# UBCMOCCA/mocca_envs

Hardware: AMD Instinct MI355X
Metric: env-steps/sec, Walker3DCustomEnv-v0 @ 4096 envs, 1/2/4/8 MI355X (higher is better)
Workload: dtype f32; 1 GPU; Walker3DCustomEnv-v0, 4096 envs/GPU, flat ground, U(-1,1) action tape, auto-reset; max_rows=48, max_contacts=12, envs_per_gpu=4096, parallelism=independent env shards x1, no collective, preroll_steps=6008

## Files before the change

mocca_envs_amd/csrc/mocca_device.h:

```cpp
#pragma once

#include <hip/hip_runtime.h>
#include <stdint.h>

#include "mocca_model.h"
#include "mocca_philox.h"
#include "topo_walker3d.h"
#include "topo_cassie.h"
#include "topo_walker2d.h"
#include "topo_crab2d.h"
#include "topo_laikago.h"

#define DI __device__ __forceinline__

#ifndef MOCCA_NS
#define MOCCA_NS mocca
#endif
#ifndef MOCCA_MAXR
#define MOCCA_MAXR 48
#endif
#ifndef MOCCA_COMPACT
#define MOCCA_COMPACT 0
#endif

// ... 11 lines not shown
#define STAMP(k) do {} while (0)
#define STAMP_BEGIN do {} while (0)
#endif

#define MOCCA_AS_CONST __attribute__((address_space(4)))
typedef const MOCCA_AS_CONST MoccaModel* ModelP;
typedef float f4_t __attribute__((ext_vector_type(4)));
typedef const MOCCA_AS_CONST f4_t* CF4P;

#ifndef MOCCA_PRIO_T3
#define MOCCA_PRIO_T3 12
#define MOCCA_PRIO_T2 7
#define MOCCA_PRIO_T1 4
#endif
constexpr int MAXR = MOCCA_MAXR;
constexpr int MAXC = MAXR >= 64 ? 20 : (MAXR >= 36 ? 12 : MAXR / 3);
constexpr bool COMPACT = MOCCA_COMPACT != 0;
constexpr bool ALT_SWEEPS = MAXR >= 64;
constexpr int DYN_STRIDE = 96;
constexpr int TERRAIN_STRIDE = 128;

#ifndef MOCCA_LDS_PAD
#define MOCCA_LDS_PAD 0
#endif
enum : int {
  L_Q = 0,
  L_QD = 24,
  L_TAU = 48,
  L_NU = 72,
  L_BASE = 100,
  L_WARM = 116,
  L_FEET = 156,
  L_PLANK = 168,
  L_JVEL = 168,
  L_Q0 = 184,
  L_V = 216,
  SVS = 20, SV_V = 6, SV_C = 12, SV_UU = 18, SV_INVD = 19,
  L_B0 = L_V + 0,
  L_SV = L_V + 48,
#if MOCCA_COMPACT
  L_ROWD = L_B0,
  L_CT = L_V + 488,
  L_P = L_CT + 16 * MAXC,
  L_M = L_P + 132,
  L_RT = L_M,
  L_GP = L_M + 264,
  GP_FLOATS = 192,
  L_OBS = L_GP,
  L_CAND = L_GP + GP_FLOATS,
  L_ABA_END = L_M + 792,
  L_A = L_V,
  L_J = L_V + 488,
  L_XL = L_V,
  L_SOLVER_END = (L_J + 28 * (MAXR + 1) > L_A + MAXR * MAXR ? L_J + 28 * (MAXR + 1) : L_A + MAXR * MAXR),
  L_TOTAL = (L_ABA_END > L_SOLVER_END ? L_ABA_END : L_SOLVER_END) + MOCCA_LDS_PAD,
#else
  L_A0 = L_V + 488,
  L_GP = L_V + 520,
  L_OBS = L_V + 520,
  L_CT = L_V + 656,
  GP_FLOATS = L_CT - L_GP,
  L_ROWD = L_CT + 16 * MAXC,
  L_RT = L_ROWD + 48,
  L_M = L_RT + 264,
  L_P = L_M + 792,
  L_ABA_END = L_P + 132,
  L_CAND = L_ABA_END,
  L_A = L_V,
  L_J = (L_V + 960 > L_RT ? L_V + 960 : L_RT),
  L_XL = L_V,
  L_TOTAL = L_V + MAXR * MAXR + 28 + MOCCA_LDS_PAD,
#endif
};
static_assert(L_ABA_END <= L_TOTAL, "ABA view must fit");
static_assert(L_SV % 4 == 0 && SVS % 4 == 0 && SVS >= 16, "joint records live in the body records, 16-byte aligned");
static_assert(L_J + (MAXR + 1) * 28 <= L_TOTAL, "Jacobian rows (+ dummy) must fit the tail of the A region");
static_assert(L_J % 4 == 0 && L_V % 4 == 0 && L_RT % 4 == 0 && L_CT % 4 == 0, "16-byte alignment of broadcast rows");
static_assert(MAXR % 2 == 0 && 3 * MAXC <= MAXR, "friction rows sit on the top 2 MAXC lanes of the row range, odd lane = second tangent");
static_assert(L_PLANK + 12 * MOCCA_MAX_PLANKS <= L_V && L_Q0 + 16 <= L_V, "persistent region overflows into the two-view region");
#if MOCCA_COMPACT
static_assert(L_TOTAL * 4 <= 8192 || MOCCA_LDS_PAD > 0, "more than 8 KB of LDS per wave: fewer than 20 waves per CU (5 per SIMD)");
static_assert(L_J >= L_SV + 22 * SVS, "J rows are written while S, V, 1/D are still being read");
static_assert(L_CAND + (MOCCA_MAX_PAIRS + 1) / 2 <= L_ABA_END && L_RT + 264 <= L_GP, "frames, geom points and the candidate list live under the link inertias");
#else
static_assert(L_TOTAL * 4 <= 10240 || MOCCA_LDS_PAD > 0 || MAXR > 48, "more than 10 KB of LDS per wave: fewer than 16 waves per CU, the 4096-env batch no longer fits one round");
static_assert(MAXR != 48 || (L_ROWD == L_V + 848 && L_RT == L_V + 896 && L_M == L_V + 1160 && L_P == L_V + 1952 && L_ABA_END == L_V + 2084 && L_J == L_V + 960), "the product's layout is unchanged");
static_assert(COMPACT || L_CAND + (MOCCA_MAX_PAIRS + 1) / 2 <= L_TOTAL, "candidate list behind the ABA view");
static_assert(L_J >= L_RT, "J rows may be written while S, U, 1/D, the factor of IA0 and the contacts are still being read");
#endif

enum : int { C_BA = 0, C_BB = 1, C_SLOT = 2, C_P = 3, C_N = 6, C_DEPTH = 9, C_MU = 10, C_ERP = 11, C_CFM = 12, C_MA = 13, C_MB = 14 };

struct StepArgs {
  const MoccaModel* model;
  float* dyn;
  uint32_t* task;
  float* terrain;
  const float* act;
  float* obs;
  float* rew;
  uint8_t* done;
  int32_t* info;
  const uint8_t* mask;
  int n_envs;
  int obs_dim;
  int auto_reset;
  int eval_mode;
  int random_pose;
  int curriculum;
  int host_retarget;
  int env_offset;
  uint32_t seed_lo, seed_hi;
  const float* curriculum_v;
  const float* eval_mode_v;
  int random_reward;
  const float* gain_v;
  float gain;
  const int32_t* inj_touch;
  const int32_t* inj_target;
  const int32_t* inj_body;
  const float* tape;
  int tape_n;
  int32_t* dbg;
  const float* traj;
  int traj_n;
  double traj_tmax, traj_cstep;
  int prio;
  const float* hf;
  int hf_rows, hf_cols;
  float hf_scale;
  float* final_obs;
  int persist_warm;
  const int32_t* order;
  int pace;
  unsigned long long* pace_acc;
  float* ep_ret;
  float* ep_masks;
  float* ep_bad;
  void* ep_rec;
  float* ep_totals;
  uint32_t ep_serial;
// ... 314 lines not shown
      L[L_SV + SVS * b + SV_UU] = L[L_TAU + b] - jdamp * L[L_QD + b];
    }
  }
}

template <class T, bool FULL>
DI void walk_kinematics(ModelP M, float* L, int lane, unsigned long long ppk) {
  asm volatile("" : "+v"(lane));
  const int b = lane < T::NB ? lane : 0;
  WalkConsts wk;
  walk_consts<FULL>(M, b, wk);
  walk_phase1<T>(L, lane, ppk);
  wsync();
  walk_phase2<T, FULL>(M, L, lane, b, ppk, wk);
}

DI void chol6_factor(const float* A, float* F) {
  float Lm[6][6];
#pragma unroll
  for (int j = 0; j < 6; ++j) {
    float s = A[sym(j, j)];
#pragma unroll
    for (int k = 0; k < j; ++k) s -= Lm[j][k] * Lm[j][k];
    const float id = rsq(s);
    F[sym(j, j)] = id;
#pragma unroll
    for (int i = j + 1; i < 6; ++i) {
      float t = A[sym(i, j)];
#pragma unroll
      for (int k = 0; k < j; ++k) t -= Lm[i][k] * Lm[j][k];
      Lm[i][j] = t * id;
      F[sym(i, j)] = Lm[i][j];
    }
  }
}
DI void chol6_solve(const float* F, const float* b, float* x) {
  float y[6];
#pragma unroll
  for (int j = 0; j < 6; ++j) {
    float t = b[j];
#pragma unroll
    for (int k = 0; k < j; ++k) t -= F[sym(j, k)] * y[k];
    y[j] = t * F[sym(j, j)];
  }
#pragma unroll
  for (int i = 5; i >= 0; --i) {
    float t = y[i];
#pragma unroll
    for (int k = i + 1; k < 6; ++k) t -= F[sym(k, i)] * x[k];
    x[i] = t * F[sym(i, i)];
  }
}

template <class T>
DI void aba_passes(ModelP M, float* L, int lane, unsigned long long ppk, float* Afac) {
  STAMP_BEGIN;
  static_assert(T::MAXW * 8 <= 64, "level does not fit a wave");
  static_assert(T::MAXW == 4 && T::MAXCH <= 4, "level pass is written for <= 4 bodies per level, <= 4 children");
  const int s = lane >> 3, i = lane & 7;
  const int ii = i < 6 ? i : 0;
  float crow[6] = {0, 0, 0, 0, 0, 0}, cpA = 0.0f;
  int bb = 0, o6i = 0, o36 = 0, osv = 0, osvi = 0;
#pragma unroll
  for (int d = T::MAXD; d >= 1; --d) {
#define MOCCA_CONT(sl) (T::clevel(d, sl) < 0 || (d < T::MAXD && T::clevel(d + 1 <= T::MAXD ? d + 1 : d, sl) == T::clevel(d, sl) + 1))
    const bool sv = s == 0 ? T::clevel(d, 0) >= 0 : s == 1 ? T::clevel(d, 1) >= 0 : s == 2 ? T::clevel(d, 2) >= 0 : s == 3 ? T::clevel(d, 3) >= 0 : false;
    const bool valid = sv && i < 6;
    if (d < T::MAXD && MOCCA_CONT(0) && MOCCA_CONT(1) && MOCCA_CONT(2) && MOCCA_CONT(3)) {
      bb -= 1; o6i -= 6; o36 -= 36; osv -= SVS; osvi -= SVS;
    } else {
      const int b = s == 0 ? T::clevel(d, 0) : s == 1 ? T::clevel(d, 1) : s == 2 ? T::clevel(d, 2) : s == 3 ? T::clevel(d, 3) : -1;
      bb = b >= 0 ? b : d;
      o6i = 6 * bb + ii; o36 = 36 * bb + 6 * ii; osv = SVS * bb; osvi = osv + ii;
    }
#undef MOCCA_CONT
    float row[6], S[6], c[6], pAi;
#pragma unroll
    for (int j = 0; j < 6; ++j) { S[j] = L[L_SV + osv + j]; c[j] = L[L_SV + osv + SV_C + j]; }
#define MOCCA_NOMASS(sl) (T::clevel(d, sl) < 0 || T::massless(T::clevel(d, sl)))
    if (MOCCA_NOMASS(0) && MOCCA_NOMASS(1) && MOCCA_NOMASS(2) && MOCCA_NOMASS(3)) {
#pragma unroll
      for (int j = 0; j < 6; ++j) row[j] = crow[j];
      pAi = cpA;
    } else {
#pragma unroll
      for (int j = 0; j < 6; ++j) row[j] = L[L_M + o36 + j] + crow[j];
      pAi = L[L_P + o6i] + cpA;
    }
#undef MOCCA_NOMASS
#pragma unroll
    for (int k = 0; k < T::MAXCH; ++k) {
#define MOCCA_LDS_CHILD(sl) (T::cchild(T::clevel(d, sl), k) != T::ccarry(T::clevel(d, sl)) ? T::cchild(T::clevel(d, sl), k) : -1)
      const int ch = s == 0 ? MOCCA_LDS_CHILD(0) : s == 1 ? MOCCA_LDS_CHILD(1) : s == 2 ? MOCCA_LDS_CHILD(2) : s == 3 ? MOCCA_LDS_CHILD(3) : -1;
      if (MOCCA_LDS_CHILD(0) >= 0 || MOCCA_LDS_CHILD(1) >= 0 || MOCCA_LDS_CHILD(2) >= 0 || MOCCA_LDS_CHILD(3) >= 0) {
        if (ch >= 0) {
#pragma unroll
          for (int j = 0; j < 6; ++j) row[j] += L[L_M + 36 * ch + 6 * ii + j];
          pAi += L[L_P + 6 * ch + ii];
        }
      }
#undef MOCCA_LDS_CHILD
    }
    const float Si = i < 6 ? L[L_SV + osvi] : 0.0f;
    const float Ui = dot6(row, S);
    float dsum = Si * Ui, psum = Si * pAi;
    group8_sum2(dsum, psum);
    float arm = L[L_SV + osv + SV_INVD], unet = L[L_SV + osv + SV_UU];
// ... 15 lines not shown
        "v_fmac_f32_dpp %4, %7, %8 quad_perm:[0,0,0,0] row_mask:0xf bank_mask:0xf\n\t"
        "v_fmac_f32_dpp %5, %7, %8 quad_perm:[1,1,1,1] row_mask:0xf bank_mask:0xf"
        : "+v"(row[0]), "+v"(row[1]), "+v"(row[2]), "+v"(row[3]), "+v"(row[4]), "+v"(row[5]) : "v"(LO), "v"(HI), "v"(nuid));
#pragma unroll
    for (int j = 0; j < 6; ++j) Iac += row[j] * c[j];
    const float pOut = pAi + Iac + uid * u;
#define MOCCA_VIA_LDS(sl) (T::clevel(d, sl) >= 0 && T::ccarry(T::parent(T::clevel(d, sl) >= 0 ? T::clevel(d, sl) : 0)) != T::clevel(d, sl))
    const bool store_m = MOCCA_VIA_LDS(0) || MOCCA_VIA_LDS(1) || MOCCA_VIA_LDS(2) || MOCCA_VIA_LDS(3);
    if (valid) {
      if (store_m) {
#pragma unroll
        for (int j = 0; j < 6; ++j) L[L_M + o36 + j] = row[j];
        L[L_P + o6i] = pOut;
      }
      L[L_SV + osvi + SV_V] = uid;
      if (i == 0) { L[L_SV + osv + SV_INVD] = id; L[L_SV + osv + SV_UU] = u * id; }
    }
#define MOCCA_NEEDZ(sl) (d > 1 && T::clevel(d - 1, sl) >= 0 && !(T::clevel(d, sl) >= 0 && !MOCCA_VIA_LDS(sl)))
    if (MOCCA_NEEDZ(0) || MOCCA_NEEDZ(1) || MOCCA_NEEDZ(2) || MOCCA_NEEDZ(3)) {
      const bool z = s == 0 ? MOCCA_NEEDZ(0) : s == 1 ? MOCCA_NEEDZ(1) : s == 2 ? MOCCA_NEEDZ(2) : MOCCA_NEEDZ(3);
#pragma unroll
      for (int j = 0; j < 6; ++j) crow[j] = z ? 0.0f : row[j];
      cpA = z ? 0.0f : pOut;
    } else {
#pragma unroll
      for (int j = 0; j < 6; ++j) crow[j] = row[j];
      cpA = pOut;
    }
#undef MOCCA_NEEDZ
#undef MOCCA_VIA_LDS
    if (store_m) wsync();
  }
  STAMP(10);
  float abase[6];
  {
    float rowb[6], pb_ = L[L_P + ii];
#pragma unroll
    for (int j = 0; j < 6; ++j) rowb[j] = L[L_M + 6 * ii + j];
#pragma unroll
    for (int k = 0; k < T::MAXCH; ++k) {
      const int ch = T::cchild(0, k);
      if (ch >= 0) {
#pragma unroll
        for (int j = 0; j < 6; ++j) rowb[j] += L[L_M + 36 * ch + 6 * ii + j];
        pb_ += L[L_P + 6 * ch + ii];
      }
    }
    if (lane < 6) {
      float4* dst = reinterpret_cast<float4*>(L + L_B0 + 8 * lane);
      dst[0] = make_float4(rowb[0], rowb[1], rowb[2], rowb[3]);
      dst[1] = make_float4(rowb[4], rowb[5], pb_, 0.0f);
    }
    wsync();
    float IA[21], pA[6];
#pragma unroll
    for (int i = 0; i < 6; ++i) {
      const float4 lo = *reinterpret_cast<const float4*>(L + L_B0 + 8 * i), hi = *reinterpret_cast<const float4*>(L + L_B0 + 8 * i + 4);
      const float rr_[6] = {lo.x, lo.y, lo.z, lo.w, hi.x, hi.y};
#pragma unroll
      for (int j = i; j < 6; ++j) IA[sym(i, j)] = rr_[j];
      pA[i] = hi.z;
    }
    float Ai[21], a0[6];
    chol6_factor(IA, Ai);
    chol6_solve(Ai, pA, a0);
#pragma unroll
    for (int i = 0; i < 21; ++i) Afac[i] = unif(Ai[i]);
#pragma unroll
    for (int i = 0; i < 6; ++i) abase[i] = -a0[i];
  }
  STAMP(11);
  {
    const int b = lane < T::NB ? lane : 0;
    float a[6], qdd = 0;
#pragma unroll
    for (int i = 0; i < 6; ++i) a[i] = abase[i];
#pragma unroll
    for (int k = 0; k < T::MAXD; ++k) {
      const int j = (int)((ppk >> (5 * k)) & 31ull);
      if (j != 0) {
        float U[6], S[6];
#pragma unroll
        for (int i = 0; i < 6; ++i) { a[i] += L[L_SV + SVS * j + SV_C + i]; U[i] = L[L_SV + SVS * j + SV_V + i]; S[i] = L[L_SV + SVS * j + i]; }
        qdd = L[L_SV + SVS * j + SV_UU] - dot6(U, a);
#pragma unroll
        for (int i = 0; i < 6; ++i) a[i] += S[i] * qdd;
      }
    }
    const float dt = M->dt;
    if (lane >= 1 && lane < T::NB) L[L_NU + 5 + b] = L[L_QD + b] + dt * qdd;
    if (lane == 0) {
      float om[3] = {L[L_BASE + 10], L[L_BASE + 11], L[L_BASE + 12]}, vl[3] = {L[L_BASE + 7], L[L_BASE + 8], L[L_BASE + 9]}, wxv[3];
      cross3(om, vl, wxv);
#pragma unroll
      for (int i = 0; i < 3; ++i) {
        L[L_NU + i] = om[i] + dt * a[i];
        L[L_NU + 3 + i] = vl[i] + dt * (a[3 + i] + wxv[i]);
      }
    }
    wsync();
  }
  STAMP(12);
}

DI void plane_space(const float* n, float* t1, float* t2) {
  if (fabsf(n[2]) > 0.70710678f) {
    const float a = n[1] * n[1] + n[2] * n[2], k = rsq(a);
    t1[0] = 0; t1[1] = -n[2] * k; t1[2] = n[1] * k;
    t2[0] = a * k; t2[1] = -n[0] * t1[2]; t2[2] = n[0] * t1[1];
  } else {
    const float a = n[0] * n[0] + n[1] * n[1], k = rsq(a);
    t1[0] = -n[1] * k; t1[1] = n[0] * k; t1[2] = 0;
    t2[0] = -n[2] * t1[1]; t2[1] = n[2] * t1[0]; t2[2] = a * k;
  }
}
DI void fast_sincos(float q, float* s, float* c);
DI void euler_to_mat(float roll, float pitch, float yaw, float* R) {
  float cr, sr, cp, sp, cy, sy;
  fast_sincos(roll, &sr, &cr); fast_sincos(pitch, &sp, &cp); fast_sincos(yaw, &sy, &cy);
  R[0] = cy * cp; R[1] = cy * sp * sr - sy * cr; R[2] = cy * sp * cr + sy * sr;
// ... 150 lines not shown
#pragma unroll 1
        for (int t = 0; t < 2; ++t) {
          const float* a = t == 0 ? v00 : v10;
          const float* b = t == 0 ? v10 : v11;
          float e1[3], e2[3], tn[3];
#pragma unroll
          for (int k = 0; k < 3; ++k) { e1[k] = b[k] - a[k]; e2[k] = v01[k] - a[k]; }
          cross3(e1, e2, tn);
          hf_triangle(C, rad, a, b, v01, tn, rsq(dot3(tn, tn)), gap, n);
        }
      }
  }
  return gap;
}
DI float hf_height_at(const float* hf, int rows, int cols, float sc, float x, float y) {
  const float ox = (float)rows / sc * 0.5f, oy = (float)cols / sc * 0.5f;
  int ix = (int)((x + ox) * sc), iy = (int)((y + oy) * sc);
  ix = ix < 0 ? 0 : (ix > cols - 1 ? cols - 1 : ix);
  iy = iy < 0 ? 0 : (iy > rows - 1 ? rows - 1 : iy);
  return hf[iy * cols + ix];
}

DI float clamp01(float x) { return x < 0.0f ? 0.0f : (x > 1.0f ? 1.0f : x); }
DI void seg_seg(const float* p1, const float* q1, const float* p2, const float* q2, float* c1, float* c2) {
  float d1[3], d2[3], r[3];
#pragma unroll
  for (int k = 0; k < 3; ++k) { d1[k] = q1[k] - p1[k]; d2[k] = q2[k] - p2[k]; r[k] = p1[k] - p2[k]; }
  const float a = dot3(d1, d1), e = dot3(d2, d2), f = dot3(d2, r), EPS = 1e-12f;
  float s, t;
  if (a <= EPS && e <= EPS) { s = t = 0; }
  else if (a <= EPS) { s = 0; t = clamp01(f * rcp(e)); }
  else {
    const float c = dot3(d1, r), ia = rcp(a);
    if (e <= EPS) { t = 0; s = clamp01(-c * ia); }
    else {
      const float b = dot3(d1, d2), den = a * e - b * b;
      s = den > EPS ? clamp01((b * f - c * e) * rcp(den)) : 0.0f;
      t = (b * s + f) * rcp(e);
      if (t < 0) { t = 0; s = clamp01(-c * ia); }
      else if (t > 1) { t = 1; s = clamp01((b - c) * ia); }
    }
  }
#pragma unroll
  for (int k = 0; k < 3; ++k) { c1[k] = p1[k] + d1[k] * s; c2[k] = p2[k] + d2[k] * t; }
}

template <class T>
DI void geom_points(ModelP M, float* L, int lane) {
  static_assert(6 * T::NG <= GP_FLOATS || (T::NPAIR == 0 && !COMPACT), "geom points would overlap the contact records read by the self-collision pass");
  if (lane < 2 * T::NG) {
    const f4_t t = *(CF4P)(M->gp_tab[lane]);
    const int b = __float_as_int(t.w);
    const float pl[3] = {t.x, t.y, t.z};
#pragma unroll
    for (int i = 0; i < 3; ++i) {
      const float4 fr = *reinterpret_cast<const float4*>(L + L_RT + 12 * b + 4 * i);
      L[L_GP + 3 * lane + i] = fr.x * pl[0] + fr.y * pl[1] + fr.z * pl[2] + fr.w;
    }
  }
}

DI void stage_planks(ModelP M, float* L, int lane, const float* ter) {
  if (lane < M->n_planks) {
    const int row = (int)ter[120 + lane];
    const float* ti = ter + 6 * row;
    float Rb[9];
    euler_to_mat(ti[4], ti[5], ti[3], Rb);
    const float cz = M->plank_com_z, dz = -M->plank_half[2] - cz;
#pragma unroll
    for (int i = 0; i < 9; ++i) L[L_PLANK + 12 * lane + i] = Rb[i];
    L[L_PLANK + 12 * lane + 9] = ti[0] + Rb[2] * dz;
    L[L_PLANK + 12 * lane + 10] = ti[1] + Rb[5] * dz;
    L[L_PLANK + 12 * lane + 11] = ti[2] + Rb[8] * dz + cz;
  }
  wsync();
}

struct HeightFieldArgs { const float* data; int rows, cols; float scale; };
struct ContactFlags { int touch0, touch1, target0, target1, touch2, touch3, body_touch, target2, target3; };
DI int cover_targets(int cover, int nsi, int n_planks, int f) { return (cover >> (4 * f + nsi % n_planks)) & 1; }

template <class T, int TASK>
DI ContactFlags collide(ModelP M, float* L, int lane, const float* ter, int next_step_index,
                        int* nc_out, int32_t* dbg, int* nc_wanted, const HeightFieldArgs hfa, int* cover_out = nullptr) {
  STAMP_BEGIN;
  const float mreach = unif(M->contact_margin);
  ContactFlags fl = {0, 0, 0, 0, 0, 0, 0, 0, 0};
  const int maxc = uni(M->max_contacts);
  bool active = false;
  float n[3] = {0, 0, 1}, P[3] = {0, 0, 0}, gap = 1e30f, mu = 0, erp = M->erp, cfm = 0;
  int body = -1, slot = lane, cover_k = -1 , gfoot = -1, gtorso = 0;
  unsigned bmask = 0u;
  if (lane < T::NSLOT) {
    const f4_t st = *(CF4P)(M->slot_tab[lane]);
    const int ids = __float_as_int(st.z);
    const int g = (ids >> 8) & 0xFF, e = (ids >> 16) & 1;
    bmask = __float_as_uint(st.w);
    if ((ids >> 25) & 1) {
      gfoot = ((ids >> 26) & 7) - 1;
      gtorso = (ids >> 29) & 1;
      float C[3], Cw[3];
      const float rad = st.x, gfric = st.y;
#pragma unroll
      for (int i = 0; i < 3; ++i) { C[i] = L[L_GP + 3 * (2 * g + e) + i]; Cw[i] = C[i] + L[L_BASE + i]; }
      body = ids & 0xFF;
      if (TASK == MOCCA_TASK_WALKER3D_PLANNER) {
        gap = sphere_heightfield(hfa.data, hfa.rows, hfa.cols, hfa.scale, Cw, rad, rad + mreach, 1 + ((ids >> 30) & 3), n);
        mu = M->plank_friction * gfric;
        const float kk = M->plank_stiffness, cc = M->plank_damping, dt = M->dt;
        const float ikc = rcp(dt * kk + cc);
// ... 81 lines not shown
      const int cover = (int)wave_or((active && gfoot >= 0 && cover_k >= 0) ? 1u << (4 * gfoot + cover_k) : 0u);
      const int npl = M->n_planks;
      fl.target0 = cover_targets(cover, next_step_index, npl, 0);
      fl.target1 = cover_targets(cover, next_step_index, npl, 1);
      if constexpr (T::NFEET > 2) { fl.target2 = cover_targets(cover, next_step_index, npl, 2); fl.target3 = cover_targets(cover, next_step_index, npl, 3); }
      if (cover_out) *cover_out = cover;
    }
    if (TASK == MOCCA_TASK_WALKER3D_PLANNER) fl.body_touch = __ballot(active && gtorso) != 0ull;
  }
  int nc = __popcll(am);
  const int n_terrain = nc;
  int n_self = 0;
  unsigned long long kept = am;
  if (nc > maxc) {
    int deeper = 0;
    for (unsigned long long mm = am; mm; mm &= mm - 1) {
      const int l = __builtin_ctzll(mm);
      const float gl = readlane(gap, l);
      deeper += (gl < gap || (gl == gap && l < lane)) ? 1 : 0;
    }
    kept = __ballot(active && deeper < maxc);
  }
  {
    const int idx = lane_rank(kept);
    if (active && ((kept >> lane) & 1ull)) {
      float* ct = L + L_CT + 16 * idx;
      ct[C_BA] = __int_as_float(body); ct[C_BB] = __int_as_float(-1); ct[C_SLOT] = __int_as_float(slot);
#pragma unroll
      for (int i = 0; i < 3; ++i) { ct[C_P + i] = P[i]; ct[C_N + i] = n[i]; }
      ct[C_DEPTH] = -gap; ct[C_MU] = mu; ct[C_ERP] = erp; ct[C_CFM] = cfm;
      ct[C_MA] = __uint_as_float(bmask); ct[C_MB] = __uint_as_float(0u);
    }
  }
  if (nc > maxc) nc = maxc;
  STAMP(13);
  const int npairs = uni(M->n_pairs);
  unsigned short* cand = reinterpret_cast<unsigned short*>(L + L_CAND);
  static_assert(2 * ((COMPACT ? L_ABA_END : L_TOTAL) - L_CAND) >= MOCCA_MAX_PAIRS, "candidate list must hold every pair");
  int ncand = 0;
#pragma unroll 1
  for (int base = 0; base < npairs; base += 64) {
    const int k = base + lane;
    bool near = false;
    if (k < npairs) {
#ifdef MOCCA_ABL_PAIRLOAD
      f4_t pt;
      pt.x = __int_as_float((k % T::NG) | (((k * 7 + 3) % T::NG) << 5) | (24 << 20)); pt.y = 0.05f; pt.z = 0.05f; pt.w = 0.04f;
#else
      const f4_t pt = *(CF4P)(M->pair_tab[k]);
#endif
      const int ids = __float_as_int(pt.x);
      const int ga = ids & 31, gb = (ids >> 5) & 31;
      float dm[3];
#pragma unroll
      for (int i = 0; i < 3; ++i)
        dm[i] = (L[L_GP + 6 * ga + i] + L[L_GP + 6 * ga + 3 + i]) - (L[L_GP + 6 * gb + i] + L[L_GP + 6 * gb + 3 + i]);
      const float reach = 2.0f * (pt.w + (float)((ids >> 20) & 0xFF) * (1.0f / 8192.0f));
      near = dot3(dm, dm) < reach * reach;
    }
    const unsigned long long nm = __ballot(near);
    if (near) cand[ncand + lane_rank(nm)] = (unsigned short)k;
    ncand += __popcll(nm);
  }
  ncand = uni(ncand);
#ifdef MOCCA_ABL_NOPASS2
  ncand = 0;
#endif
  wsync();
#pragma unroll 1
  for (int base = 0; base < ncand; base += 64) {
    bool hit = false;
    float nn[3] = {0, 0, 0}, PP[3] = {0, 0, 0}, g2 = 0, mu2 = 0;
    int ba = -1, bb = -1;
    if (base + lane < ncand) {
      const int k = cand[base + lane];
      const f4_t pt = *(CF4P)(M->pair_tab[k]);
      const int ids = __float_as_int(pt.x);
      const int ga = ids & 31, gb = (ids >> 5) & 31;
      float a1[3], a2[3], b1[3], b2[3];
#pragma unroll
      for (int i = 0; i < 3; ++i) {
        a1[i] = L[L_GP + 6 * ga + i]; a2[i] = L[L_GP + 6 * ga + 3 + i];
        b1[i] = L[L_GP + 6 * gb + i]; b2[i] = L[L_GP + 6 * gb + 3 + i];
      }
      float ca[3], cb[3];
      seg_seg(a1, a2, b1, b2, ca, cb);
      float d[3] = {ca[0] - cb[0], ca[1] - cb[1], ca[2] - cb[2]};
      const float d2 = dot3(d, d), id = rsq(d2), dist = d2 * id, ra = pt.y, rb = pt.z;
      g2 = dist - ra - rb;
      hit = g2 < (float)((ids >> 20) & 0xFF) * (1.0f / 8192.0f) && d2 > 1e-18f;
#ifdef MOCCA_ABL_NOHITS
      hit = hit && g2 < -1e30f;
#endif
      if (hit) {
#pragma unroll
        for (int i = 0; i < 3; ++i) {
          nn[i] = d[i] * id;
          PP[i] = 0.5f * ((ca[i] - ra * d[i] * id) + (cb[i] + rb * d[i] * id));
        }
        ba = (ids >> 10) & 31; bb = (ids >> 15) & 31;
        mu2 = M->g_friction[ga] * M->g_friction[gb];
      }
    }
    const unsigned long long hm = __ballot(hit);
    if (TASK == MOCCA_TASK_WALKER3D_PLANNER && hm != 0ull) {
      int tor = 0;
      if (hit) { const int ids2 = __float_as_int((*(CF4P)(M->pair_tab[cand[base + lane]])).x); tor = M->g_torso[ids2 & 31] | M->g_torso[(ids2 >> 5) & 31]; }
      if (__ballot(hit && tor) != 0ull) fl.body_touch = 1;
    }
// ... 265 lines not shown
enum : int { L_T0 = L_BASE + 13, L_PACE = L_BASE + 14, L_KEEPWARM = L_BASE + 15  };
constexpr unsigned PACE_CNT_BITS = 24, PACE_WINDOW = 128;
DI void pace_start(const StepArgs& a, float* L, int lane, int pace) {
  if (lane == 0) {
    int p16 = pace >> PACE_TICK_SHIFT;
    if (pace < 0) {
      const unsigned long long v = __hip_atomic_load(a.pace_acc, __ATOMIC_RELAXED, __HIP_MEMORY_SCOPE_AGENT);
      const unsigned cnt = (unsigned)v & ((1u << PACE_CNT_BITS) - 1u);
      p16 = cnt > 0u ? (int)((float)(v >> PACE_CNT_BITS) / (float)cnt * (float)(-pace) * 0.0625f) : 0;
    }
    L[L_PACE] = __int_as_float(p16);
    if (pace != 0) L[L_T0] = __uint_as_float((unsigned)__builtin_amdgcn_s_memtime());
  }
}
DI void pace_finish(const StepArgs& a, const float* L, int lane, int pace) {
  if (pace < 0 && lane == 0 && (blockIdx.x % 61u) == 0u) {
    const unsigned el = ((unsigned)__builtin_amdgcn_s_memtime() - __float_as_uint(L[L_T0])) >> PACE_TICK_SHIFT;
    const unsigned long long old = atomicAdd(a.pace_acc, ((unsigned long long)el << PACE_CNT_BITS) | 1ull);
    if (((unsigned)old & ((1u << PACE_CNT_BITS) - 1u)) + 1u == PACE_WINDOW) {
      const unsigned long long sum = (old >> PACE_CNT_BITS) + el;
      atomicAdd(a.pace_acc, 0ull - (((sum >> 1) << PACE_CNT_BITS) | (unsigned long long)(PACE_WINDOW / 2)));
    }
  }
}
DI bool pace_on(const float* L) { return uni(__float_as_int(L[L_PACE])) > 0; }
DI void pace_checkpoint(const float* L, int done, int total) {
  const unsigned p16 = (unsigned)uni(__float_as_int(L[L_PACE]));
  if (p16 == 0u) return;
  const unsigned el = (unsigned)__builtin_amdgcn_s_memtime() - (unsigned)uni(__float_as_int(L[L_T0]));
  const unsigned lhs = (el >> PACE_TICK_SHIFT) * (unsigned)total, r = p16 * (unsigned)done;
  if (lhs > r + (r >> MOCCA_PACE_SHIFT)) __builtin_amdgcn_s_setprio(3);
  else if (lhs > r) __builtin_amdgcn_s_setprio(2);
  else if (lhs > r - (r >> MOCCA_PACE_SHIFT)) __builtin_amdgcn_s_setprio(1);
  else __builtin_amdgcn_s_setprio(0);
}
DI void dbg_fold_step(int32_t* dbg, int lane) {
  if (dbg && lane == 0) {
    unsigned long long h = ((unsigned long long)(unsigned)dbg[17] << 32) | (unsigned)dbg[16];
#pragma unroll 1
    for (int w = 0; w < 12; ++w) h = (h ^ (unsigned long long)(unsigned)dbg[w]) * 0x9E3779B97F4A7C15ull;
    dbg[16] = (int32_t)(unsigned)h; dbg[17] = (int32_t)(unsigned)(h >> 32); dbg[18] += 1;
  }
}
template <class T, bool MATRIX_PIPE>
DI void solve_constraints(ModelP M, float* L, int lane, int nc_found, int nc_wanted, unsigned long long ppk, int32_t* dbg, const float* Afac, int prio, int& rows_out) {
  const int wave_flags = uni(__float_as_int(L[L_KEEPWARM]));
  const bool keep_warm = (wave_flags & 1) != 0;
  STAMP_BEGIN;
  const float dt = unif(M->dt), idt = rcp(dt);
  const int maxr = uni(M->max_rows);
  int nl;
  {
    bool act = false;
    if (lane < 2 * T::NJ) {
      const int b = 1 + (lane >> 1), side = lane & 1;
      const float q = L[L_Q + b];
      const float gap = side == 0 ? q - M->jlo[b] : M->jhi[b] - q;
      const float vel = (side == 0 ? 1.0f : -1.0f) * L[L_NU + 5 + b];
      act = M->limit_at_violation ? !(gap > 0.0f) : gap + dt * vel < M->limit_slack;
    }
    const unsigned long long lm = __ballot(act);
    const int rk = lane_rank(lm);
    if (act && rk < maxr) reinterpret_cast<int*>(L)[L_ROWD + rk] = lane;
    nl = uni(__popcll(lm));
    if (dbg && lane == 0) {
      dbg[5] = (int32_t)(unsigned)lm; dbg[6] = (int32_t)(unsigned)(lm >> 32);
      const int nfix = 3 * T::NCLOS + ((T::NCLOS > 0 && M->planar) ? 3 : 0), mc = M->max_contacts;
      const int wanted = nl + nfix + 3 * nc_wanted;
      dbg[12] += nc_wanted > mc ? 1 : 0;
      dbg[13] += nl + nfix + 3 * (nc_wanted < mc ? nc_wanted : mc) > maxr ? 1 : 0;
      dbg[14] += 1;
      if (wanted > dbg[15]) dbg[15] = wanted;
    }
    if (nl > maxr) nl = maxr;
  }
  constexpr int NCL = 3 * T::NCLOS;
  const int NFIX = NCL + ((T::NCLOS > 0 && uni(M->planar)) ? 3 : 0);
  int nc = uni(nc_found);
  if (nc > (maxr - nl - NFIX) / 3) nc = (maxr - nl - NFIX) / 3;
  if (nc < 0) nc = 0;
  const int nr = nl + NFIX + 3 * nc;
  if (dbg && lane == 0) { dbg[0] = nr; dbg[1] = nl; dbg[2] = nc; }
  if (!pace_on(L)) set_issue_priority(nr, prio);
  rows_out = nr;
  wsync();
  STAMP(16);
  if (nr == 0) {
    if (dbg && lane == 0) { dbg[8] = 0; dbg[9] = 0; dbg[10] = 0; dbg[11] = 0; }
    if (keep_warm && lane < T::NSLOT) L[L_WARM + lane] = 0.0f;
    wsync();
    return;
  }
  const int r = lane;
  const int r_fr = nl + NFIX + nc;
  const int row_gap = MAXR - nr;
  const bool is_fric = r >= MAXR - 2 * nc && r < MAXR;
  const bool has_row = r < r_fr || is_fric;
  const int ci = is_fric ? (MAXR - 1 - r) >> 1 : r - nl - NFIX;
  int kind = -1, ba = 0, bb = -1, jl = -1, slot = -1;
  float F[6] = {0, 0, 0, 0, 0, 0}, sgn = 0, bias = 0, cfm = 0, lam = 0, mu = 0;
  float F2[6] = {0, 0, 0, 0, 0, 0};
  if (r < nl) {
    const int c = reinterpret_cast<int*>(L)[L_ROWD + r];
    const int b = 1 + (c >> 1), side = c & 1;
    const float q = L[L_Q + b];
    const float gap = side == 0 ? q - M->jlo[b] : M->jhi[b] - q;
    kind = 0; jl = b; ba = b; sgn = side == 0 ? 1.0f : -1.0f;
    bias = gap < 0 ? M->erp_noncontact * (-gap) * idt : -gap * idt;
  } else if (T::NCLOS > 0 && r < nl + NCL) {
    const int c = (r - nl) / 3, ax = (r - nl) % 3;
    ba = M->cl_body_a[c]; bb = M->cl_body_b[c];
    kind = 3;
    float Pa[3], Pb[3], Ra[9], Rb[9], la[3], lb[3];
#pragma unroll
    for (int x = 0; x < 9; ++x) { Ra[x] = L[L_RT + 12 * ba + 4 * (x / 3) + x % 3]; Rb[x] = L[L_RT + 12 * bb + 4 * (x / 3) + x % 3]; }
#pragma unroll
    for (int x = 0; x < 3; ++x) { la[x] = M->cl_point_a[c][x]; lb[x] = M->cl_point_b[c][x]; }
    matvec3(Ra, la, Pa); matvec3(Rb, lb, Pb);
#pragma unroll
    for (int x = 0; x < 3; ++x) { Pa[x] += L[L_RT + 12 * ba + 4 * x + 3]; Pb[x] += L[L_RT + 12 * bb + 4 * x + 3]; }
    float dir[3] = {ax == 0 ? 1.0f : 0.0f, ax == 1 ? 1.0f : 0.0f, ax == 2 ? 1.0f : 0.0f}, pn[3];
    cross3(Pa, dir, pn);
#pragma unroll
    for (int x = 0; x < 3; ++x) { F[x] = pn[x]; F[3 + x] = dir[x]; }
    cross3(Pb, dir, pn);
#pragma unroll
    for (int x = 0; x < 3; ++x) { F2[x] = pn[x]; F2[3 + x] = dir[x]; }
    const float e = ax == 0 ? Pb[0] - Pa[0] : (ax == 1 ? Pb[1] - Pa[1] : Pb[2] - Pa[2]);
    bias = M->erp_noncontact * e * idt;
  } else if (T::NCLOS > 0 && r < nl + NFIX) {
    const int k = r - nl - NCL;
    const int comp = k == 0 ? 0 : (k == 1 ? 2 : 4);
    kind = 3; ba = 0; bb = -1;
#pragma unroll
    for (int x = 0; x < 6; ++x) F[x] = x == comp ? 1.0f : 0.0f;
    const float err = k == 0 ? L[L_RT + 9]  : (k == 1 ? -L[L_RT + 1]  : L[L_BASE + 1] - M->init_pos[1]);
    bias = -M->erp_noncontact * err * idt;
  } else if (has_row) {
    const float* ct = L + L_CT + 16 * ci;
    float n[3] = {ct[C_N], ct[C_N + 1], ct[C_N + 2]}, P[3] = {ct[C_P], ct[C_P + 1], ct[C_P + 2]}, dir[3];
    ba = __float_as_int(ct[C_BA]); bb = __float_as_int(ct[C_BB]);
    if (!is_fric) {
      kind = 1;
      dir[0] = n[0]; dir[1] = n[1]; dir[2] = n[2];
      const float depth = ct[C_DEPTH] - unif(M->linear_slop);
      bias = depth > 0 ? ct[C_ERP] * depth * idt : depth * idt;
      cfm = ct[C_CFM];
      slot = __float_as_int(ct[C_SLOT]);
      const float wsf = unif(M->warmstart);
      lam = (wsf != 0.0f && slot >= 0) ? wsf * L[L_WARM + slot] : 0.0f;
    } else {
      kind = 2;
      float t1[3], t2[3];
      plane_space(n, t1, t2);
      const bool second = (r & 1) != 0;
#pragma unroll
      for (int x = 0; x < 3; ++x) dir[x] = second ? t2[x] : t1[x];
      mu = ct[C_MU];
    }
// ... 306 lines not shown
    matmul3(jr, Rq, Tl);
    float4* rec = reinterpret_cast<float4*>(L + L_SV + SVS * j);
    rec[0] = make_float4(Tl[0], Tl[1], Tl[2], Tl[3]);
    rec[1] = make_float4(Tl[4], Tl[5], Tl[6], Tl[7]);
    rec[2] = make_float4(Tl[8], M->jpos[j][0], M->jpos[j][1], M->jpos[j][2]);
    rec[3] = make_float4(ax[0], ax[1], ax[2], L[L_QD + j]);
  }
  wsync();
}

template <class T, int TASK>
DI ContactFlags substep(ModelP M, float* L, int lane, const float* ter, int next_step_index,
                        unsigned long long ppk, int32_t* dbg, int prio, int& rows_out,
                        const HeightFieldArgs hfa = HeightFieldArgs{nullptr, 0, 0, 0.0f}, int sidx = 0, int nsub = 1, int* cover_out = nullptr) {
  const int per0 = 64 + MOCCA_PACE_ROWUNIT * rows_out, done0 = sidx * per0, total = nsub * per0;
  STAMP(30);
  stage_joints<T>(M, L, lane);
  STAMP(29);
  int nc = 0, nc_wanted = 0;
  float Afac[21] = {0, 0, 0, 0, 0, 0, 0, 0, 0, 0, 0, 0, 0, 0, 0, 0, 0, 0, 0, 0, 0};
  ContactFlags fl = {0, 0, 0, 0, 0, 0, 0, 0, 0};
  if constexpr (COMPACT) {
    static_assert(!COMPACT || T::NCLOS == 0, "closure rows read the body frames after the ABA: not in the compact layout");
    int wl = lane;
    asm volatile("" : "+v"(wl));
    walk_phase1<T>(L, wl, ppk);
    wsync();
    STAMP(0);
    geom_points<T>(M, L, lane);
    wsync();
    STAMP(15);
#ifndef MOCCA_SKIP_COLLIDE
    fl = collide<T, TASK>(M, L, lane, ter, next_step_index, &nc, dbg, &nc_wanted, hfa, cover_out);
#endif
    wsync();
    const int wb = wl < T::NB ? wl : 0;
    WalkConsts wk;
    walk_consts<true>(M, wb, wk);
    walk_phase2<T, true>(M, L, wl, wb, ppk, wk);
    wsync();
  } else {
    walk_kinematics<T, true>(M, L, lane, ppk);
    wsync();
    STAMP(0);
    geom_points<T>(M, L, lane);
    wsync();
    STAMP(15);
#ifndef MOCCA_SKIP_COLLIDE
    fl = collide<T, TASK>(M, L, lane, ter, next_step_index, &nc, dbg, &nc_wanted, hfa, cover_out);
#endif
  }
  STAMP(1);
  pace_checkpoint(L, done0 + 20, total);
#ifndef MOCCA_SKIP_ABA
  aba_passes<T>(M, L, lane, ppk, Afac);
#endif
  STAMP(2);
  pace_checkpoint(L, done0 + 36, total);
#ifndef MOCCA_SKIP_SOLVE
  solve_constraints<T, (COMPACT || MAXR != 48 || TASK != MOCCA_TASK_WALKER3D_PLANNER)>(M, L, lane, nc, nc_wanted, ppk, dbg, Afac, prio, rows_out);
#endif
  if (dbg) { __builtin_amdgcn_s_waitcnt(0); dbg_fold_step(dbg, lane); }
  STAMP(3);
#ifdef MOCCA_DUMMY_VALU
  {
    float x = (float)lane;
#ifdef MOCCA_DUMMY_ILP
    float y = x + 1.0f, z = x + 2.0f, u = x + 3.0f;
#pragma unroll 1
    for (int i = 0; i < MOCCA_DUMMY_VALU; ++i) { x = fmaf(x, 1.0001f, 0.5f); y = fmaf(y, 0.9999f, -0.5f); z = fmaf(z, 1.0001f, 0.5f); u = fmaf(u, 0.9999f, -0.5f); }
    asm volatile("" :: "v"(y), "v"(z), "v"(u));
#else
#pragma unroll 1
    for (int i = 0; i < MOCCA_DUMMY_VALU; ++i) { x = fmaf(x, 1.0001f, 0.5f); x = fmaf(x, 0.9999f, -0.5f); x = fmaf(x, 1.0001f, 0.5f); x = fmaf(x, 0.9999f, -0.5f); }
#endif
    asm volatile("" :: "v"(x));
  }
#endif
  integrate<T>(M, L, lane);
  STAMP(4);
  pace_checkpoint(L, (sidx + 1) * (64 + MOCCA_PACE_ROWUNIT * rows_out), nsub * (64 + MOCCA_PACE_ROWUNIT * rows_out));
  return fl;
}

DI void quat_to_rpy(const float* q, float* rpy) {
  const float x = q[0], y = q[1], z = q[2], w = q[3];
  const float sarg = -2 * (x * z - w * y);
  if (sarg <= -0.99999f) { rpy[1] = -1.5707963267948966f; rpy[0] = 0; rpy[2] = 2 * atan2f(x, -y); }
  else if (sarg >= 0.99999f) { rpy[1] = 1.5707963267948966f; rpy[0] = 0; rpy[2] = 2 * atan2f(-x, y); }
  else {
    rpy[0] = atan2f(2 * (y * z + w * x), w * w - x * x - y * y + z * z);
    rpy[1] = asinf(sarg);
    rpy[2] = atan2f(2 * (x * y + w * z), w * w + x * x - y * y - z * z);
  }
}

DI void quat_to_rp_heading(const float* q, float* rp, float* cy, float* sy) {
  const float x = q[0], y = q[1], z = q[2], w = q[3];
  const float sarg = -2 * (x * z - w * y);
  if (sarg <= -0.99999f) { rp[1] = -1.5707963267948966f; rp[0] = 0; const float yaw = 2 * atan2f(x, -y); *cy = cosf(yaw); *sy = sinf(yaw); }
  else if (sarg >= 0.99999f) { rp[1] = 1.5707963267948966f; rp[0] = 0; const float yaw = 2 * atan2f(-x, y); *cy = cosf(yaw); *sy = sinf(yaw); }
  else {
    rp[0] = atan2f(2 * (y * z + w * x), w * w - x * x - y * y + z * z);
    rp[1] = asinf(sarg);
    const float A = 2 * (x * y + w * z), B = w * w + x * x - y * y - z * z, n = rsq(A * A + B * B);
    *cy = B * n; *sy = A * n;
  }
}

template <class T> constexpr int ROBOT_OBS = 6 + 2 * T::NJ + T::NFEET;
struct RobotObs { float rpy[3];  float cy, sy; int jal; float spd; float height; bool finite; };

template <class T>
// ... 445 lines not shown
```

Before: 41.80 million env-steps/s.

## Split base Cholesky across lanes, cache geom midpoints and joint-limit gaps

Three trims to the per-step path. The 6x6 base inertia Cholesky is now done column-per-lane with readlane broadcasts instead of redundantly on every lane. Geometry-point pair midpoints are precomputed with DPP adds into aligned LDS records for the broad-phase test. Joint-limit gaps are stored in LDS during row detection so the solver does not recompute them from q and the model limits. These add LDS footprint and readlane serialization, and use inline DPP asm that assumes adjacent-lane pairing of geom points.

```diff
diff --git a/mocca_envs_amd/csrc/mocca_device.h b/mocca_envs_amd/csrc/mocca_device.h
--- a/mocca_envs_amd/csrc/mocca_device.h
+++ b/mocca_envs_amd/csrc/mocca_device.h
@@ -87,6 +87,8 @@
   L_A = L_V,
   L_J = L_V + 488,
   L_XL = L_V,
+  L_MID = L_CAND + (MOCCA_MAX_PAIRS + 1) / 2,
+  L_LGAP = L_ABA_END - MAXR,
   L_SOLVER_END = (L_J + 28 * (MAXR + 1) > L_A + MAXR * MAXR ? L_J + 28 * (MAXR + 1) : L_A + MAXR * MAXR),
   L_TOTAL = (L_ABA_END > L_SOLVER_END ? L_ABA_END : L_SOLVER_END) + MOCCA_LDS_PAD,
 #else
@@ -104,6 +106,8 @@
   L_A = L_V,
   L_J = (L_V + 960 > L_RT ? L_V + 960 : L_RT),
   L_XL = L_V,
+  L_MID = L_CAND + (MOCCA_MAX_PAIRS + 1) / 2,
+  L_LGAP = L_GP,
   L_TOTAL = L_V + MAXR * MAXR + 28 + MOCCA_LDS_PAD,
 #endif
 };
@@ -122,6 +126,17 @@
 static_assert(MAXR != 48 || (L_ROWD == L_V + 848 && L_RT == L_V + 896 && L_M == L_V + 1160 && L_P == L_V + 1952 && L_ABA_END == L_V + 2084 && L_J == L_V + 960), "the product's layout is unchanged");
 static_assert(COMPACT || L_CAND + (MOCCA_MAX_PAIRS + 1) / 2 <= L_TOTAL, "candidate list behind the ABA view");
 static_assert(L_J >= L_RT, "J rows may be written while S, U, 1/D, the factor of IA0 and the contacts are still being read");
+static_assert(L_LGAP + MAXR <= L_CT && L_J >= L_CT, "limit gaps: written after the collision pass, read before the first J row or A entry is stored");
+#endif
+#if MOCCA_COMPACT
+static_assert(L_LGAP >= L_J + 28 * (MAXR + 1) && L_LGAP >= L_A + MAXR * MAXR && L_LGAP >= L_M && L_LGAP + MAXR <= L_TOTAL, "limit gaps: behind the solver view, in the dead link inertias");
+#endif
+static_assert(L_MID % 4 == 0 && L_MID >= L_CAND + (MOCCA_MAX_PAIRS + 1) / 2, "midpoint records: 16-byte aligned, behind the candidate list");
+template <class T>
+#ifdef MOCCA_NO_TRIM_1
+constexpr bool MID_RECORDS = false;
+#else
+constexpr bool MID_RECORDS = T::NPAIR > 0 && 6 * T::NG <= GP_FLOATS && L_MID + 4 * T::NG <= (COMPACT ? (int)L_ABA_END : (int)L_TOTAL);
 #endif
 
 enum : int { C_BA = 0, C_BB = 1, C_SLOT = 2, C_P = 3, C_N = 6, C_DEPTH = 9, C_MU = 10, C_ERP = 11, C_CFM = 12, C_MA = 13, C_MB = 14 };
@@ -542,7 +557,7 @@
   }
 }
 
-template <class T>
+template <class T, bool FACTOR_ACROSS_LANES>
 DI void aba_passes(ModelP M, float* L, int lane, unsigned long long ppk, float* Afac) {
   STAMP_BEGIN;
   static_assert(T::MAXW * 8 <= 64, "level does not fit a wave");
@@ -664,20 +679,44 @@
       dst[1] = make_float4(rowb[4], rowb[5], pb_, 0.0f);
     }
     wsync();
-    float IA[21], pA[6];
-#pragma unroll
-    for (int i = 0; i < 6; ++i) {
-      const float4 lo = *reinterpret_cast<const float4*>(L + L_B0 + 8 * i), hi = *reinterpret_cast<const float4*>(L + L_B0 + 8 * i + 4);
-      const float rr_[6] = {lo.x, lo.y, lo.z, lo.w, hi.x, hi.y};
-#pragma unroll
-      for (int j = i; j < 6; ++j) IA[sym(i, j)] = rr_[j];
-      pA[i] = hi.z;
-    }
-    float Ai[21], a0[6];
-    chol6_factor(IA, Ai);
-    chol6_solve(Ai, pA, a0);
-#pragma unroll
-    for (int i = 0; i < 21; ++i) Afac[i] = unif(Ai[i]);
+    float a0[6];
+#ifdef MOCCA_NO_TRIM_3
+    constexpr bool across = false;
+#else
+    constexpr bool across = FACTOR_ACROSS_LANES;
+#endif
+    if constexpr (across) {
+      const int li = lane < 6 ? lane : 0;
+      float colA[6], pA[6], own[6];
+#pragma unroll
+      for (int j = 0; j < 6; ++j) { colA[j] = L[L_B0 + 8 * j + li]; pA[j] = L[L_B0 + 8 * j + 6]; }
+#pragma unroll
+      for (int j = 0; j < 6; ++j) {
+        float t = colA[j];
+#pragma unroll
+        for (int k = 0; k < j; ++k) t -= own[k] * Afac[sym(j, k)];
+        Afac[sym(j, j)] = readlane(rsq(t), j);
+        own[j] = t * Afac[sym(j, j)];
+#pragma unroll
+        for (int i = j + 1; i < 6; ++i) Afac[sym(i, j)] = readlane(own[j], i);
+      }
+      chol6_solve(Afac, pA, a0);
+    } else {
+      float IA[21], pA[6];
+#pragma unroll
+      for (int i = 0; i < 6; ++i) {
+        const float4 lo = *reinterpret_cast<const float4*>(L + L_B0 + 8 * i), hi = *reinterpret_cast<const float4*>(L + L_B0 + 8 * i + 4);
+        const float rr_[6] = {lo.x, lo.y, lo.z, lo.w, hi.x, hi.y};
+#pragma unroll
+        for (int j = i; j < 6; ++j) IA[sym(i, j)] = rr_[j];
+        pA[i] = hi.z;
+      }
+      float Ai[21];
+      chol6_factor(IA, Ai);
+      chol6_solve(Ai, pA, a0);
+#pragma unroll
+      for (int i = 0; i < 21; ++i) Afac[i] = unif(Ai[i]);
+    }
 #pragma unroll
     for (int i = 0; i < 6; ++i) abase[i] = -a0[i];
   }
@@ -934,10 +973,21 @@
     const f4_t t = *(CF4P)(M->gp_tab[lane]);
     const int b = __float_as_int(t.w);
     const float pl[3] = {t.x, t.y, t.z};
+    float pw[3];
 #pragma unroll
     for (int i = 0; i < 3; ++i) {
       const float4 fr = *reinterpret_cast<const float4*>(L + L_RT + 12 * b + 4 * i);
-      L[L_GP + 3 * lane + i] = fr.x * pl[0] + fr.y * pl[1] + fr.z * pl[2] + fr.w;
+      pw[i] = fr.x * pl[0] + fr.y * pl[1] + fr.z * pl[2] + fr.w;
+      L[L_GP + 3 * lane + i] = pw[i];
+    }
+    if constexpr (MID_RECORDS<T>) {
+      float m0, m1, m2;
+      asm("s_nop 1\n\t"
+          "v_add_f32_dpp %0, %3, %3 quad_perm:[1,0,3,2] row_mask:0xf bank_mask:0xf\n\t"
+          "v_add_f32_dpp %1, %4, %4 quad_perm:[1,0,3,2] row_mask:0xf bank_mask:0xf\n\t"
+          "v_add_f32_dpp %2, %5, %5 quad_perm:[1,0,3,2] row_mask:0xf bank_mask:0xf"
+          : "=&v"(m0), "=&v"(m1), "=&v"(m2) : "v"(pw[0]), "v"(pw[1]), "v"(pw[2]));
+      if (!(lane & 1)) *reinterpret_cast<float4*>(L + L_MID + 2 * lane) = make_float4(m0, m1, m2, 0.0f);
     }
   }
 }
@@ -1125,9 +1175,14 @@
       const int ids = __float_as_int(pt.x);
       const int ga = ids & 31, gb = (ids >> 5) & 31;
       float dm[3];
-#pragma unroll
-      for (int i = 0; i < 3; ++i)
-        dm[i] = (L[L_GP + 6 * ga + i] + L[L_GP + 6 * ga + 3 + i]) - (L[L_GP + 6 * gb + i] + L[L_GP + 6 * gb + 3 + i]);
+      if constexpr (MID_RECORDS<T>) {
+        const float4 sa_ = *reinterpret_cast<const float4*>(L + L_MID + 4 * ga), sb_ = *reinterpret_cast<const float4*>(L + L_MID + 4 * gb);
+        dm[0] = sa_.x - sb_.x; dm[1] = sa_.y - sb_.y; dm[2] = sa_.z - sb_.z;
+      } else {
+#pragma unroll
+        for (int i = 0; i < 3; ++i)
+          dm[i] = (L[L_GP + 6 * ga + i] + L[L_GP + 6 * ga + 3 + i]) - (L[L_GP + 6 * gb + i] + L[L_GP + 6 * gb + 3 + i]);
+      }
       const float reach = 2.0f * (pt.w + (float)((ids >> 20) & 0xFF) * (1.0f / 8192.0f));
       near = dot3(dm, dm) < reach * reach;
     }
@@ -1499,16 +1554,22 @@
   int nl;
   {
     bool act = false;
+    float gap = 0.0f;
     if (lane < 2 * T::NJ) {
       const int b = 1 + (lane >> 1), side = lane & 1;
       const float q = L[L_Q + b];
-      const float gap = side == 0 ? q - M->jlo[b] : M->jhi[b] - q;
+      gap = side == 0 ? q - M->jlo[b] : M->jhi[b] - q;
       const float vel = (side == 0 ? 1.0f : -1.0f) * L[L_NU + 5 + b];
       act = M->limit_at_violation ? !(gap > 0.0f) : gap + dt * vel < M->limit_slack;
     }
     const unsigned long long lm = __ballot(act);
     const int rk = lane_rank(lm);
-    if (act && rk < maxr) reinterpret_cast<int*>(L)[L_ROWD + rk] = lane;
+    if (act && rk < maxr) {
+      reinterpret_cast<int*>(L)[L_ROWD + rk] = lane;
+#ifndef MOCCA_NO_TRIM_2
+      L[L_LGAP + rk] = gap;
+#endif
+    }
     nl = uni(__popcll(lm));
     if (dbg && lane == 0) {
       dbg[5] = (int32_t)(unsigned)lm; dbg[6] = (int32_t)(unsigned)(lm >> 32);
@@ -1550,8 +1611,12 @@
   if (r < nl) {
     const int c = reinterpret_cast<int*>(L)[L_ROWD + r];
     const int b = 1 + (c >> 1), side = c & 1;
+#ifndef MOCCA_NO_TRIM_2
+    const float gap = L[L_LGAP + r];
+#else
     const float q = L[L_Q + b];
     const float gap = side == 0 ? q - M->jlo[b] : M->jhi[b] - q;
+#endif
     kind = 0; jl = b; ba = b; sgn = side == 0 ? 1.0f : -1.0f;
     bias = gap < 0 ? M->erp_noncontact * (-gap) * idt : -gap * idt;
   } else if (T::NCLOS > 0 && r < nl + NCL) {
@@ -1964,13 +2029,14 @@
   }
   STAMP(1);
   pace_checkpoint(L, done0 + 20, total);
+  constexpr bool PLANNER48 = !COMPACT && MAXR == 48 && TASK == MOCCA_TASK_WALKER3D_PLANNER;
 #ifndef MOCCA_SKIP_ABA
-  aba_passes<T>(M, L, lane, ppk, Afac);
+  aba_passes<T, !PLANNER48>(M, L, lane, ppk, Afac);
 #endif
   STAMP(2);
   pace_checkpoint(L, done0 + 36, total);
 #ifndef MOCCA_SKIP_SOLVE
-  solve_constraints<T, (COMPACT || MAXR != 48 || TASK != MOCCA_TASK_WALKER3D_PLANNER)>(M, L, lane, nc, nc_wanted, ppk, dbg, Afac, prio, rows_out);
+  solve_constraints<T, !PLANNER48>(M, L, lane, nc, nc_wanted, ppk, dbg, Afac, prio, rows_out);
 #endif
   if (dbg) { __builtin_amdgcn_s_waitcnt(0); dbg_fold_step(dbg, lane); }
   STAMP(3);
```

Result: faster. 42.41 million env-steps/s, median of 6 (+1.5%).
